# IvanBanny/para-ortho-pca-bo

Hardware: AMD Instinct MI355X
Metric: BO iterations/sec (incl. GP refit + EI opt), BBOB f15 d=40 (higher is better)
Workload: dtype f64; 1 GPU; configs[1]: PCA_BO on BBOB f15 d=40, budget=450, n_DoE=120, EI, var_threshold=0.95; one run per GPU (run list f15/d40/instances 0..N-1 partitioned by pcabo.sharding), timed steps spread evenly over the 330 BO iterations of the run; num_restarts=10, raw_samples=512, batch_limit=5, maxiter=200, parallelism=run-parallel x1

## Files before the change

### para-ortho-pca-bo_amd/csrc/kernels_acq.hip

```cpp
#include "pcabo_internal.h"
#include <algorithm>
#include <cstdlib>
#include <mutex>

#define PSTRIDE (2 + 2 * PCABO_MAXD)

#ifdef PCABO_ACQ_TIMING
__device__ unsigned long long g_acq_stamps[16];
#define STAMP(i) do { if (blockIdx.x == gridDim.x / 2 && blockIdx.y == 0 && threadIdx.x == 0) g_acq_stamps[i] = wall_clock64(); } while (0)
#define STAMP_FIN(i) do { if (blockIdx.y == 0 && threadIdx.x == 0) g_acq_stamps[i] = wall_clock64(); } while (0)
extern "C" int pcabo_debug_acq_stamps(unsigned long long* out16) {
  return hipMemcpyFromSymbol(out16, HIP_SYMBOL(g_acq_stamps), sizeof(g_acq_stamps)) == hipSuccess ? 0 : -3;
}
#else
#define STAMP(i)
#define STAMP_FIN(i)
#endif

__device__ inline void st_wt(double* p, double v) {
  __hip_atomic_store(p, v, __ATOMIC_RELAXED, __HIP_MEMORY_SCOPE_AGENT);
}

template <int SLAB>
__device__ inline int slab_row(int s, int m, int NP) {
// ... 23 lines not shown
    for (int t = 0; t < 8; ++t) {
      const int si = sl + 3 * t;
      const int sc = si < S ? si : 0;
      a[t] = base[(size_t)sc * PSTRIDE + 2 + c];
      b[t] = base[(size_t)sc * PSTRIDE + 2 + PCABO_MAXD + c];
    }
#pragma unroll
    for (int t = 0; t < 8; ++t) { if (sl + 3 * t < S) { gs += a[t]; gm += b[t]; } }
  }
  *gs_out = gs;
  *gm_out = gm;
}

__device__ void acq_finish_scalar(const double* base, int S, int q, const double* ystats, const AcqParams& p, double* val,
                                  double* host_val, double* coef, int lane);
__device__ void acq_scalar_core(double vv, double mus, int q, double ym, double ysd, const AcqParams& p, double* val,
                                double* host_val, double* coef, int l);
template <int SLAB>
__device__ inline void acq_tail(int combine, double* s_v, double* partial, unsigned int* counters, int q, int S, int k,
                                const double* bounds4, const double* ystats, const AcqParams& prm, double* val,
                                double* grad, double* host_val, double* host_grad, HostMirror* hm,
                                unsigned long long seq, int tid, int w, int l) {
  if (!combine) return;
  int* s_flag = reinterpret_cast<int*>(s_v + SLAB);
  STAMP(6);
  asm volatile("s_waitcnt vmcnt(0)" ::: "memory");
  __syncthreads();
  STAMP(7);
  if (tid == 0) {
    unsigned int t = __hip_atomic_fetch_add(&counters[q], 1u, __ATOMIC_RELAXED, __HIP_MEMORY_SCOPE_AGENT);
    int last = ((t % (unsigned int)S) == (unsigned int)(S - 1));
    if (last) {
// ... 56 lines not shown
    counters = zrun(counters, ab.zs, run_); val = zrun(val, ab.zs, run_); grad = zrun(grad, ab.zs, run_);        \
    Xq = zrun(Xq, ab.xq_host ? ab.hzs : ab.zs, run_);                                                            \
    host_val = zrun(host_val, ab.hzs, run_); host_grad = zrun(host_grad, ab.hzs, run_); hm = zrun(hm, ab.hzs, run_); \
    if (ab.k_dev) k = *zrun(ab.k_dev, ab.zs, run_);                                                              \
    if (ab.bestf) prm.best_f = *zrun(ab.bestf, ab.zs, run_);                                                     \
  }                                                                                                              \
  (void)qsel_;

template <int SLAB>
__global__ __launch_bounds__(256) void k_acq_fused(
    QueryArgs qa, const double* __restrict__ Xq, int q_total, int n, int k, int NP, int ld,
    const double* __restrict__ ZnT, const double* __restrict__ R, const double* __restrict__ alpha,
    const double* __restrict__ bounds4, const double* __restrict__ ystats, AcqParams prm, double* partial,
    unsigned int* counters, double* __restrict__ val, double* __restrict__ grad,
    double* host_val, double* host_grad, HostMirror* hm, unsigned long long seq, int combine, int ,
    MailPair* , MailPair* , AcqBatch ab) {
  ACQ_BATCH_PROLOGUE()
  const double inv_ls = prm.inv_ls;
  const int kernel = prm.kernel, want_grad = prm.want_grad;
  extern __shared__ __attribute__((aligned(16))) double s_dyn[];
  double* s_ks = s_dyn;
  double* s_cf = s_dyn + NP;
  double* s_tm = s_dyn + 2 * NP;
  double* s_xn = s_dyn + 3 * NP;
  double* s_v = s_xn + PCABO_MAXD;
  const int tid = threadIdx.x, w = tid >> 6, l = tid & 63;
  const int s = blockIdx.x, q = ab.table ? qsel_ : (int)blockIdx.y, S = gridDim.x;
  double* out = partial + ((size_t)q * S + s) * PSTRIDE;
  STAMP(0);

  if (tid < k) {
// ... 98 lines not shown
    if (l == 0) {
#pragma unroll
      for (int u = 0; u < 8; ++u) {
        const int c = c0 + w + 4 * u;
        if (c < k) { st_wt(out + 2 + c, gs[u]); st_wt(out + 2 + PCABO_MAXD + c, gm[u]); }
      }
    }
  }
  }

  acq_tail<SLAB>(combine, s_v, partial, counters, q, S, k, bounds4, ystats, prm, val, grad, host_val, host_grad, hm, seq, tid, w, l);
}

#define FIN_STAGE_PER_WAVE (11 * 2 * 40)
__device__ inline bool acq_server_finisher(const MailPair* rec, int S, int k, int q, unsigned long long seq,
                                           const double* ystats, const AcqParams& prm, double* val, double* grad,
                                           double* host_val, double* host_grad, HostMirror* hm, double rng_c,
                                           double* s_fin, double* s_coef, double* s_stage, int* s_srv,
                                           unsigned long long t0, int w, int l) {
  if (w == 0) {
    const double ym = ystats[0], ysd = ystats[1];
    const void* ptr[8];
    pcabo_u4 o[8];
    const MailPair* mine = rec + (size_t)(l < S ? l : 0) * PSTRIDE;
#pragma unroll
    for (int t = 0; t < 8; ++t) ptr[t] = mine + (t & 1);
    for (;;) {
      ld_pairs_sys8(ptr, o);
      const bool ok = pair_tag(o[0]) == seq && pair_tag(o[1]) == seq;
      if (__all(ok)) break;
      if (__any(wall_clock64() - t0 > PCABO_SERVER_TIMEOUT_TICKS)) { if (l == 0) *s_srv = 1; break; }
      __builtin_amdgcn_s_sleep(1);
    }
    double vm[2] = {l < S ? pair_value(o[0]) : 0.0, l < S ? pair_value(o[1]) : 0.0};
    wave_sum_multi<2>(vm, l);
    constexpr int lane_vv = wave_multi_lane(2, 0), lane_mus = wave_multi_lane(2, 1);
    const double vv = read_lane(vm[0], lane_vv), mus = read_lane(vm[0], lane_mus);
    acq_scalar_core(vv, mus, q, ym, ysd, prm, val, host_val, s_coef, l);
  } else if (prm.want_grad) {
    const int first = w - 1;
    const int ns = first < S ? (S - first + 2) / 3 : 0;
    const int total = ns * 2 * k;
    double* stage = s_stage + (size_t)(w - 1) * FIN_STAGE_PER_WAVE;
    for (int i0 = 0; i0 < total; i0 += 512) {
      const void* ptr[8];
      int item[8];
#pragma unroll
      for (int t = 0; t < 8; ++t) {
        const int i = i0 + l + 64 * t;
        item[t] = i < total ? i : -1;
        const int ii = i < total ? i : 0;
        const int st = ii / (2 * k), rem = ii - st * 2 * k, which = rem >= k, c = rem - which * k;
        ptr[t] = rec + (size_t)(first + 3 * st) * PSTRIDE + 2 + which * PCABO_MAXD + c;
      }
// ... 11 lines not shown
      for (int t = 0; t < 8; ++t) if (item[t] >= 0) stage[item[t]] = pair_value(o[t]);
    }
    __builtin_amdgcn_fence(__ATOMIC_RELEASE, "wavefront");
    __builtin_amdgcn_wave_barrier();
    __builtin_amdgcn_fence(__ATOMIC_ACQUIRE, "wavefront");
    if (l < k) {
      double gs = 0.0, gm = 0.0;
      for (int st = 0; st < ns; ++st) { gs += stage[st * 2 * k + l]; gm += stage[st * 2 * k + k + l]; }
      s_fin[(w - 1) * 2 * PCABO_MAXD + l] = gs;
      s_fin[(w - 1) * 2 * PCABO_MAXD + PCABO_MAXD + l] = gm;
    }
  }
  __syncthreads();
  if (*s_srv) return false;
  if (w == 0) {
    if (prm.want_grad && l < k) {
      const double c_mu = s_coef[0], c_sg = s_coef[1];
      const double gs = (s_fin[l] + s_fin[2 * PCABO_MAXD + l]) + s_fin[4 * PCABO_MAXD + l];
      const double gm = (s_fin[PCABO_MAXD + l] + s_fin[3 * PCABO_MAXD + l]) + s_fin[5 * PCABO_MAXD + l];
      const double g = __fma_rn(c_mu, gm, c_sg * gs) / rng_c;
      grad[(size_t)q * k + l] = g;
      if (host_grad) host_grad[(size_t)q * k + l] = g;
    }
    if (hm && l == 0)
      __hip_atomic_store(const_cast<unsigned long long*>(&hm->qflag[q]), seq, __ATOMIC_RELEASE, __HIP_MEMORY_SCOPE_SYSTEM);
  }
  return true;
}

#define FIN_LDS_DOUBLES (6 * PCABO_MAXD + 2 + 3 * FIN_STAGE_PER_WAVE + 2)
__device__ __noinline__ void acq_server_finish_main(double* s_mem, MailPair* dev_mail,
                                                    int ctrl_idx, const MailPair* part_pairs, int S, int k, int q,
                                                    const double* __restrict__ bounds4, const double* __restrict__ ystats,
                                                    const AcqParams& prm, double* val, double* grad, double* host_val,
                                                    double* host_grad, HostMirror* hm, unsigned long long seq) {
  double* s_fin = s_mem;
  int* s_srvp = reinterpret_cast<int*>(s_mem + FIN_LDS_DOUBLES - 1);
  const int tid = threadIdx.x, l = tid & 63;
  const int w = __builtin_amdgcn_readfirstlane(tid >> 6);
  double rng_c = 1.0;
  if (tid < k) rng_c = bounds4[PCABO_MAXD + tid] - bounds4[tid];
  for (unsigned long long cur_seq = seq;; ++cur_seq) {
    const unsigned long long t0 = wall_clock64();
    if (tid == 0) { s_srvp[0] = 0; s_srvp[1] = 0; }
    __syncthreads();
    if (w == 0) {
      for (;;) {
        const pcabo_u4 hd = ld_pair_sys(dev_mail + ctrl_idx);
        if (__all(mail_seq(hd) == cur_seq)) { if (pair_value(hd) == 0.0 && l == 0) *s_srvp = 1; break; }
        if (__any(wall_clock64() - t0 > PCABO_SERVER_TIMEOUT_TICKS)) { if (l == 0) *s_srvp = 1; break; }
        __builtin_amdgcn_s_sleep(1);
      }
    }
    __syncthreads();
    if (*s_srvp) return;
    if (!acq_server_finisher(part_pairs + (size_t)q * S * PSTRIDE, S, k, q, cur_seq, ystats, prm, val, grad, host_val,
                             host_grad, hm, rng_c, s_fin, s_fin + 6 * PCABO_MAXD, s_fin + 6 * PCABO_MAXD + 2, s_srvp, t0, w, l))
      return;
    __syncthreads();
  }
}

#define ACQ_SLAB32_NP 448
int acq_slabs(int NP) { return NP / (NP >= ACQ_SLAB32_NP ? 32 : 16); }

template <int NU, int CU>
__device__ inline void publish_grad(const double (&gs)[CU], const double (&gm)[CU], int w, int k, int l, MailPair* pout,
                                    double* out, unsigned long long seq) {
  static_assert(NU <= CU, "components per wave");
  double v[2 * NU];
#pragma unroll
  for (int u = 0; u < NU; ++u) { v[2 * u] = gs[u]; v[2 * u + 1] = gm[u]; }
// ... 2 lines not shown
  const int c = w + 4 * (i >> 1);
  if (i >= 0 && c < k) {
    const int off = 2 + (i & 1) * PCABO_MAXD + c;
    if (pout) st_pair_sys(pout + off, make_pair(v[0], seq));
    else st_wt(out + off, v[0]);
  }
}

template <int SLAB, int NB, bool SRV>
__global__ __launch_bounds__(256) void k_acq_fast(
    QueryArgs qa, const double* __restrict__ Xq, int q_total, int n, int k, int NP_rt, int ld,
    const double* __restrict__ ZnT, const double* __restrict__ R, const double* __restrict__ alpha,
    const double* __restrict__ bounds4, const double* __restrict__ ystats, AcqParams prm, double* partial,
    unsigned int* counters, double* __restrict__ val, double* __restrict__ grad,
    double* host_val, double* host_grad, HostMirror* hm, unsigned long long seq, int combine, int qb,
    MailPair* dev_mail, MailPair* part_pairs, AcqBatch ab) {
  if (!SRV) { ACQ_BATCH_PROLOGUE() }
  constexpr int NP = NB * 64;
  constexpr int CU = 10;
  constexpr int RW = SLAB / 4;
  constexpr int NM = (NB + 3) / 4;
  const double inv_ls = prm.inv_ls;
  const int kernel = prm.kernel, want_grad = prm.want_grad;
  extern __shared__ __attribute__((aligned(16))) double s_dyn[];
  double* s_ks = s_dyn;
  double* s_cf = s_dyn + NP;
  double* s_tm = s_dyn + 2 * NP;
  double* s_xn = s_dyn + 3 * NP;
  double* s_v = s_xn + PCABO_MAXD;
  double* s_p4 = s_v + SLAB + 2;
  const int tid = threadIdx.x, l = tid & 63;
  const int w = __builtin_amdgcn_readfirstlane(tid >> 6);
  constexpr bool server = SRV;
  const int s = blockIdx.x, S = server ? (int)gridDim.x - 1 : (int)gridDim.x;
  if (server && s == S) {
    acq_server_finish_main(s_dyn, dev_mail, 1 + q_total * k + (int)blockIdx.y, part_pairs, S, k,
                           blockIdx.y, bounds4, ystats, prm, val, grad, host_val, host_grad, hm, seq);
    return;
  }
  STAMP(0);

  double z[CU][NB], r[RW][NB], al[NM];
  const unsigned lane8 = (unsigned)l * 8u;
#pragma unroll
  for (int u = 0; u < CU; ++u) {
    const int c = w + 4 * u;
    const char* zr = reinterpret_cast<const char*>(ZnT + (size_t)c * ld);
#pragma unroll
    for (int b = 0; b < NB; ++b) {
      z[u][b] = 0.0;
      if (c < k) z[u][b] = *reinterpret_cast<const double*>(zr + lane8 + 512 * b);
    }
// ... 205 lines not shown
    return;
  }
  double log_phi = -0.5 * (u * u + log2pi);
  if (u > -1e6) {
    const double ex = erfcx(-inv_sqrt2 * u);
    const double E = (ex * fabs(u)) * 1.2533141373155003;
    *h = log_phi + log1p(-E);
    const double dw = (u + 0.7978845608028654 / ex) + 1.0 / u;
    *dh = -u - dw * E / (1.0 - E);
  } else {
    *h = log_phi - 2.0 * log(fabs(u));
    *dh = -u - 2.0 / u;
  }
}

__device__ void acq_scalar_core(double vv, double mus, int q, double ym, double ysd, const AcqParams& p, double* val,
                                double* host_val, double* coef, int l) {
  const double mu = ym + ysd * mus;
  double var = (1.0 - vv) * (ysd * ysd);
  bool clamped = false;
  if (!(var >= 1e-10)) { var = 1e-10; clamped = true; }
  if (var < 1e-12) { var = 1e-12; clamped = true; }
  const double sigma = sqrt(var);
  double u = (mu - p.best_f) / sigma;
  const double sgn = p.maximize ? 1.0 : -1.0;
  u *= sgn;
  double value, dv_du, dv_dsig;
  if (p.acq == 0) {
    double h, dh;
    log_ei_helper(u, &h, &dh);
    value = h + log(sigma);
    dv_du = dh;
    dv_dsig = 1.0 / sigma;
  } else {
    value = 0.5 * erfc(-0.7071067811865476 * u);
    dv_du = 0.3989422804014327 * exp(-0.5 * u * u);
    dv_dsig = 0.0;
  }
  if (l == 0) {
    val[q] = value;
    if (host_val) host_val[q] = value;
    coef[0] = dv_du * sgn * ysd / sigma;
    coef[1] = clamped ? 0.0 : (dv_dsig - dv_du * u / sigma) * (-(ysd * ysd) / sigma);
  }
  STAMP_FIN(12);
}

__device__ void acq_finish_scalar(const double* base, int S, int q, const double* ystats, const AcqParams& p, double* val,
                                  double* host_val, double* coef, int l) {
  const double ym = ystats[0], ysd = ystats[1];
  double vv = 0.0, mus = 0.0;
  for (int s = l; s < S; s += 64) { vv += base[(size_t)s * PSTRIDE]; mus += base[(size_t)s * PSTRIDE + 1]; }
  vv = wave_sum(vv);
  mus = wave_sum(mus);
  STAMP_FIN(11);
  acq_scalar_core(vv, mus, q, ym, ysd, p, val, host_val, coef, l);
}

__device__ void acq_finish_query(const double* base, int S, int k, int q, const double* bounds4, const double* ystats,
                                 const AcqParams& p, double* val, double* grad, double* host_val, double* host_grad,
// ... 572 lines not shown
bool acq_server_possible(int q, int n, int k, int NP) {
  static int cus = -1;
  if (cus < 0) {
    int dev = 0;
    if (hipGetDevice(&dev) != hipSuccess || hipDeviceGetAttribute(&cus, hipDeviceAttributeMultiprocessorCount, dev) != hipSuccess) cus = 0;
  }
  if (k > 40 || NP > 512 || q < 1 || q > PCABO_INLAUNCH_MAXQ || (size_t)q * k > PCABO_QA_MAX) return false;
  const int S = acq_slabs(NP);
  return (S + 1) * q <= cus && S <= 32;
}

void launch_acq(hipStream_t st, const QueryArgs* qa, const double* Xq, int q, int n, int k, int NP, int ld,
                const double* ZnT, const double* R, const double* alpha, const double* bounds4, const double* ystats,
                AcqParams p, double* partial, unsigned int* counters, double* val,
                double* grad, double* host_val, double* host_grad, HostMirror* hm, unsigned long long seq,
                MailPair* dev_mail, MailPair* part_pairs, AcqBatch ab, int B,
                int table_entries) {
  const int slab = NP >= ACQ_SLAB32_NP ? 32 : 16;
  const int S = NP / slab;
  static const QueryArgs empty = {};
  const int combine = hm != nullptr;
  const int nb = NP / 64;
  const bool fast = k <= 40 && nb <= 8;
  const int qb = (fast && !combine && q >= 64) ? 8 : 1;
  const int gy = ab.table ? table_entries : (q + qb - 1) / qb;
  const int gz = ab.table ? 1 : B;
#define ACQ_ARGS qa ? *qa : empty, Xq, q, n, k, NP, ld, ZnT, R, alpha, bounds4, ystats, p, partial, counters, val, grad, \
                 host_val, host_grad, hm, seq, combine, qb, dev_mail, part_pairs, ab
  const int FIN_LDS = 6 * PCABO_MAXD + 2;
#define ACQ_LDS(SL, NBV) (3 * NBV * 64 + PCABO_MAXD + SL + 2 + (4 * NBV * 64 > FIN_LDS ? 4 * NBV * 64 : FIN_LDS))
#define ACQ_FAST(SL, NBV)                                                                                      \
  case NBV:                                                                                                    \
    if (dev_mail)                                                                                              \
      hipLaunchKernelGGL((k_acq_fast<SL, NBV, true>), dim3(S + 1, gy), dim3(256),                              \
                         (size_t)std::max<int>(ACQ_LDS(SL, NBV), FIN_LDS_DOUBLES) * sizeof(double), st, ACQ_ARGS); \
    else                                                                                                       \
      hipLaunchKernelGGL((k_acq_fast<SL, NBV, false>), dim3(S, gy, gz), dim3(256),                             \
                         (size_t)ACQ_LDS(SL, NBV) * sizeof(double), st, ACQ_ARGS);                             \
    break;
  if (fast) {
    if (slab == 16) {
      switch (nb) { ACQ_FAST(16, 1) ACQ_FAST(16, 2) ACQ_FAST(16, 3) ACQ_FAST(16, 4) ACQ_FAST(16, 5) ACQ_FAST(16, 6)
                    ACQ_FAST(16, 7) ACQ_FAST(16, 8) }
// ... 59 lines not shown
```

### para-ortho-pca-bo_amd/csrc/pcabo_api.hip

```cpp
#include "../../include/pcabo.h"
#include "pcabo_internal.h"
#include "lbfgsb.h"
#include "host_side.h"

#include <algorithm>
#include <atomic>
#include <chrono>
#include <thread>
#include <condition_variable>
#include <functional>
#include <mutex>
#include <cstdlib>
#include <cmath>
#include <cstdio>
#include <cstring>
#include <new>
#include <vector>
#include <dirent.h>
#include <fcntl.h>
#include <signal.h>
#include <stdint.h>
#include <cerrno>
#include <unistd.h>
#include <emmintrin.h>
// ... 73 lines not shown
  unsigned int* dCounters = nullptr;
  int cnt_S = 0; bool cnt_dirty = true;
  double* dKS = nullptr;
  double* dBestF = nullptr;
  double* dMll = nullptr;
  char *dRegion = nullptr, *hRegion = nullptr;
  size_t region_bytes = 0, hregion_bytes = 0;
  bool in_batch = false; int batch_index = 0;
  bool rt_stale = false;
  HostMirror* hm = nullptr;
  double *hXq = nullptr, *hVal = nullptr, *hGrad = nullptr, *hSmall = nullptr, *hBestF = nullptr;
  double* hMll = nullptr;
  MailPair* dMail = nullptr;
  bool mail_bar = false;
  MailPair* dPairs = nullptr;
  bool opt_resident = true;
  bool opt_group_acq = false;
  bool bestf_f32 = true;
  int srv_penalty = 0;
  unsigned long long seq = 0;
  OptHelper helper;
  std::vector<std::unique_ptr<OptHelper>> more_helpers;
  bool registered = false;
  bool alone = true; int alone_age = 0;
  char err[512] = {0};
  bool prof = false;
  std::vector<ProfPair> pairs;
  size_t pairs_used = 0;
  double prof_ms[PROF_GROUPS] = {0};
  double prof_pair_ms = 0.0;
// ... 265 lines not shown
    HIPCHK(hipHostMalloc((void**)&ctx->hRegion, ctx->hregion_bytes, hipHostMallocDefault));
    memset(ctx->hRegion, 0, ctx->hregion_bytes);
  }
  carve_device(ctx, ctx->dRegion);
  carve_host(ctx, ctx->hRegion);
  if (!dreg) {
    HIPCHK(hipMemsetAsync(ctx->dRegion, 0, ctx->region_bytes, ctx->stream));
    if (hipExtMallocWithFlags((void**)&ctx->dMail, PCABO_MAIL_PAIRS * sizeof(MailPair), hipDeviceMallocFinegrained) != hipSuccess) {
      (void)hipGetLastError();
      HIPCHK(dalloc(&ctx->dMail, PCABO_MAIL_PAIRS));
    }
    HIPCHK(hipMemsetAsync(ctx->dMail, 0, PCABO_MAIL_PAIRS * sizeof(MailPair), ctx->stream));
    const size_t np = (size_t)PCABO_INLAUNCH_MAXQ * 32 * (2 + 2 * PCABO_MAXD);
    HIPCHK(dalloc(&ctx->dPairs, np));
    HIPCHK(hipMemsetAsync(ctx->dPairs, 0, np * sizeof(MailPair), ctx->stream));
    HIPCHK(hipStreamSynchronize(ctx->stream));
    ctx->mail_bar = mail_bar_usable(ctx);
  } else {
    ctx->opt_resident = false;
  }
  {
    static std::atomic<unsigned long long> ctx_counter{0};
    ctx->seq = ((unsigned long long)(getpid() & 0xffff) << 44) + ((ctx_counter.fetch_add(1) + 1) << 30);
  }
  return PCABO_OK;
}

static void ctx_teardown(pcabo_ctx* ctx) {
  (void)hipSetDevice(ctx->device);
  if (ctx->stream) (void)hipStreamSynchronize(ctx->stream);
  for (auto& p : ctx->pairs) { (void)hipEventDestroy(p.a); (void)hipEventDestroy(p.b); }
  if (!ctx->in_batch) {
    if (ctx->dRegion) (void)hipFree(ctx->dRegion);
    if (ctx->hRegion) (void)hipHostFree(ctx->hRegion);
    if (ctx->dMail) (void)hipFree(ctx->dMail);
    if (ctx->dPairs) (void)hipFree(ctx->dPairs);
  }
  if (ctx->evBounds) (void)hipEventDestroy(ctx->evBounds);
  if (ctx->evPca) (void)hipEventDestroy(ctx->evPca);
  if (ctx->stream && !ctx->in_batch) (void)hipStreamDestroy(ctx->stream);
  ctx->helper.shutdown();
  for (auto& h : ctx->more_helpers) h->shutdown();
  ctx->more_helpers.clear();
  if (ctx->registered) presence_unregister(ctx->device);
}

static bool ctx_sizes_ok(int max_n, int max_d, int max_q) {
  return max_n >= 2 && max_d >= 1 && max_d <= PCABO_MAXD && max_q >= 1 && max_q < PCABO_CNT_DONE;
}

extern "C" {
// ... 559 lines not shown
  memcpy(val, ctx->hVal, (size_t)q * sizeof(double));
  return PCABO_OK;
}

int pcabo_logei(pcabo_ctx* ctx, const double* Xq, int q, double best_f, int maximize, double* val, double* grad) {
  return pcabo_acq_eval(ctx, Xq, q, best_f, maximize, PCABO_ACQ_LOG_EI, val, grad);
}

static void server_post(pcabo_ctx* ctx, int cap, int nq, int k, unsigned long long tag) {
  MailPair* m = ctx->dMail;
  const int np = cap * k;
  for (int i = 0; i < np; ++i) put_mail_pair(m + 1 + i, ctx->hXq[i], tag);
  for (int q = 0; q < cap; ++q) put_mail_pair(m + 1 + np + q, q < nq ? 1.0 : 0.0, tag);
  _mm_sfence();
}
static int server_wait(pcabo_ctx* ctx, int nq, unsigned long long tag) {
  if (wait_flags(ctx->hm, 0, nq, tag, deadline_in(3)) != FLAGS_SET)
    return set_err(ctx, PCABO_ERR_TIMEOUT, "resident acquisition kernel did not answer%s", "");
  return PCABO_OK;
}

int pcabo_optimize_acqf(pcabo_ctx* ctx, const double* ics, int num_restarts, int batch_limit, const double* bounds,
                        int maxiter, double best_f, int maximize, int acq, double* cand, double* vals, int* info,
                        int* failed) {
  if (!ctx) return PCABO_ERR_ARG;
  if (!ics || !bounds || !cand || !vals || num_restarts < 1 || batch_limit < 1 || num_restarts > ctx->max_q ||
      (acq != PCABO_ACQ_LOG_EI && acq != PCABO_ACQ_PI))
    return set_err(ctx, PCABO_ERR_ARG, "pcabo_optimize_acqf: bad argument%s", "");
  if (!ctx->have_gp) return set_err(ctx, PCABO_ERR_ARG, "pcabo_optimize_acqf: call pcabo_gp_condition first%s", "");
  HIPCHK(hipSetDevice(ctx->device));
  const int k = ctx->k;
  RunRestarts run;
// ... 45 lines not shown
    for (int gi = 0; gi < ngroups; ++gi) {
      qoff[gi] = -1;
      if (!grp[gi].active) continue;
      qoff[gi] = nq;
      memcpy(ctx->hXq + (size_t)nq * k, grp[gi].x.data(), grp[gi].x.size() * sizeof(double));
      nq += grp[gi].nq;
    }
    if (nq == 0) break;
    int rc;
    if (round_no == 1 && (ctx->alone_age++ & 7) == 0) ctx->alone = presence_alone(ctx->device);
    const bool only_context_here = presence_local_contexts(ctx->device) == 1;
    if (round_no == 1 && ctx->srv_penalty > 0) --ctx->srv_penalty;
    else if (round_no == 1 && ctx->opt_resident && ctx->mail_bar && !ctx->opt_group_acq && ctx->alone && only_context_here && !ctx->prof && acq_server_possible(nq, ctx->n, k, ctx->NP)) {
      srv_cap = nq;
      launch_acq(ctx->stream, nullptr, nullptr, srv_cap, ctx->n, k, ctx->NP, ctx->ld, ctx->dZnT, ctx->dR, ctx->dAlpha,
                 ctx->dBounds4, ctx->dYstats, p, ctx->dPartial, ctx->dCounters, ctx->dVal, ctx->dGrad, ctx->hVal, ctx->hGrad,
                 ctx->hm, ctx->seq + 1, ctx->dMail, ctx->dPairs);
      HIPCHK(hipGetLastError());
      if (ngroups == 2 && grp[0].active && grp[1].active && nq == num_restarts) {
        const unsigned long long seq0 = ctx->seq;
        MailPair* m = ctx->dMail;
        const int cap = srv_cap;
        std::atomic<int> abort_flag{0};
        int timed_out[2] = {0, 0}, got_nan[2] = {0, 0}, left[2] = {0, 0}, slow_first[2] = {0, 0};
        unsigned long long used[2] = {0, 0};
        auto free_loop = [&](int gi) {
          RestartGroup& rg = grp[gi];
          const int q0 = rg.q0, nqg = rg.nq;
          unsigned long long r = 0;
          for (;;) {
            if (abort_flag.load(std::memory_order_relaxed)) { pending[gi] = 1; break; }
            const unsigned long long tag = seq0 + (++r);
            for (int t = 0; t < nqg * k; ++t) put_mail_pair(m + 1 + q0 * k + t, rg.x[t], tag);
            for (int j = 0; j < nqg; ++j) put_mail_pair(m + 1 + cap * k + q0 + j, 1.0, tag);
            _mm_sfence();
            const auto t0 = std::chrono::steady_clock::now();
            unsigned long spins = 0;
            bool ok = true;
            for (int j = 0; j < nqg && ok; ++j) {
              while (__atomic_load_n(&ctx->hm->qflag[q0 + j], __ATOMIC_ACQUIRE) != tag) {
                if ((++spins & 0xFFF) == 0) {
                  if (abort_flag.load(std::memory_order_relaxed)) { ok = false; break; }
                  if (std::chrono::steady_clock::now() - t0 > std::chrono::seconds(3)) {
                    timed_out[gi] = 1; abort_flag.store(1, std::memory_order_relaxed); ok = false; break;
                  }
                }
              }
            }
            if (!ok) { pending[gi] = 1; break; }
            if (r == 1 && std::chrono::steady_clock::now() - t0 > std::chrono::milliseconds(1)) slow_first[gi] = 1;
            if (!rg.absorb(ctx->hVal, ctx->hGrad, q0)) { got_nan[gi] = 1; abort_flag.store(1, std::memory_order_relaxed); break; }
            if (!rg.advance()) break;
          }
          const unsigned long long bye = seq0 + r + 1;
          for (int j = 0; j < nqg; ++j) put_mail_pair(m + 1 + cap * k + q0 + j, 0.0, bye);
          _mm_sfence();
          left[gi] = 1;
          used[gi] = r + 1;
        };
        hp.fn = [&] { free_loop(1); };
        const unsigned fticket = hp.go.load(std::memory_order_relaxed) + 1;
        hp.go.store(fticket, std::memory_order_release);
        free_loop(0);
        while (hp.done.load(std::memory_order_acquire) != fticket) __builtin_ia32_pause();
        hp.fn = [&] { for (int gi = 1; gi < ngroups; gi += T) advance(gi); };
        HIPCHK(hipStreamSynchronize(ctx->stream));
        ctx->seq = seq0 + std::max(used[0], used[1]) + 1;
        srv_cap = 0;
        if (got_nan[0] || got_nan[1]) return set_err(ctx, PCABO_ERR_NAN, "NaN in acquisition gradient%s", "");
        if (timed_out[0] || timed_out[1]) ctx->srv_penalty = 1000;
        else if (slow_first[0] || slow_first[1]) ctx->srv_penalty = 40;
        if (!grp[0].active && !grp[1].active) break;
        continue;
      }
    }
    if (srv_cap > 0) {
      const unsigned long long tag = ++ctx->seq;
      const double tp = now();
      server_post(ctx, srv_cap, nq, k, tag);
      rc = server_wait(ctx, nq, tag);
      if (rc == PCABO_ERR_TIMEOUT) {
        server_stop.stop();
        ctx->srv_penalty = 1000;
        rc = eval_staged(ctx, nq, p);
      } else if (round_no == 1 && now() - tp > 1e-3) {
        ctx->srv_penalty = 40;
      }
    } else if (group_mode(ctx, nq, 1) && batch_limit <= PCABO_GROUP_Q && ngroups <= 8) {
      int g0[8], gn[8], ng = 0;
      for (int gi = 0; gi < ngroups; ++gi) if (qoff[gi] >= 0) { g0[ng] = qoff[gi]; gn[ng] = grp[gi].nq; ++ng; }
      rc = eval_staged_groups(ctx, g0, gn, ng, p);
    } else {
      rc = eval_staged(ctx, nq, p);
    }
    if (rc != PCABO_OK) return rc;
// ... 548 lines not shown
  const int B = batch->B, kmax = batch_max_k(batch);
  pcabo_ctx* c0 = batch->ctx[0];
  if (phase != 2) {
  for (int b = 0; b < B; ++b)
    memcpy(batch->ctx[b]->hXq, Xq + (size_t)b * q * batch->max_d, (size_t)q * batch->ctx[b]->k * sizeof(double));
  BHIPCHK(hipMemcpy2DAsync(c0->dXq, batch->zs, c0->hXq, batch->hzs, (size_t)q * kmax * sizeof(double), B, hipMemcpyHostToDevice, s));
  int rc = batch_put_best_f(batch, best_f);
  if (rc != PCABO_OK) return rc;
  AcqParams p = make_params(c0, 0.0, maximize, acq, 0);
  p.inv_ls = 1.0 / batch->lengthscale; p.kernel = batch->kernel;
  if (score_gemm_possible(q))
    launch_score(s, c0->dXq, q, batch->n, kmax, batch->NP, c0->ld, c0->dZnT, c0->dR, c0->dAlpha, c0->dBounds4, c0->dYstats, p,
                 c0->dKS, c0->dPartial, c0->dVal, batch_ab(batch, 0, 0), B);
  else
    launch_acq(s, nullptr, c0->dXq, q, batch->n, kmax, batch->NP, c0->ld, c0->dZnT, c0->dR, c0->dAlpha, c0->dBounds4, c0->dYstats,
               p, c0->dPartial, c0->dCounters, c0->dVal, c0->dGrad, nullptr, nullptr, nullptr, 0, nullptr, nullptr,
               batch_ab(batch, 0, 0), B, 0);
  BHIPCHK(hipMemcpy2DAsync(c0->hVal, batch->hzs, c0->dVal, batch->zs, (size_t)q * sizeof(double), B, hipMemcpyDeviceToHost, s));
  BHIPCHK(hipGetLastError());
  batch->score_enqueued = true;
  }
  if (phase == 1) return PCABO_OK;
  BHIPCHK(wait_stream(s));
  BHIPCHK(hipGetLastError());
  batch->score_enqueued = false;
  batch->gp_pending = false; batch->have_gp = true;
  int worst = PCABO_OK;
  for (int b = 0; b < B; ++b) {
    pcabo_ctx* c = batch->ctx[b];
    int st = PCABO_OK;
    if (c->hm->chol_info != 0) {
// ... 243 lines not shown
    QueryArgs tab;
    unsigned* ent = reinterpret_cast<unsigned*>(tab.x);
    int nent = 0;
    auto launch = [&](const AcqParams& p, bool groups) -> bool {
      const unsigned long long seq = batch->seq.fetch_add(1) + 1;
      const int n = nent;
      nent = 0;
      if (groups) {
        if (launch_acq_group(st, &tab, n, c0->hXq, batch->n, kmax, batch->NP, c0->ld, c0->dZnT, c0->dR, c0->dAlpha,
                             c0->dBounds4, c0->dYstats, p, c0->dPartial, c0->dCounters + PCABO_GROUP_CNT_OFFSET, c0->dVal,
                             c0->dGrad, c0->hVal, c0->hGrad, c0->hm, seq, batch_ab(batch, 1, 1)) != 0)
          return false;
      } else {
        launch_acq(st, &tab, c0->hXq, PCABO_INLAUNCH_MAXQ, batch->n, kmax, batch->NP, c0->ld, c0->dZnT, c0->dR,
                   c0->dAlpha, c0->dBounds4, c0->dYstats, p, c0->dPartial, c0->dCounters, c0->dVal, c0->dGrad, c0->hVal,
                   c0->hGrad, c0->hm, seq, nullptr, nullptr, batch_ab(batch, 1, 1), B, n);
      }
      if (hipGetLastError() != hipSuccess) return false;
      const auto deadline = deadline_in(20);
      for (int e = 0; e < n; ++e) {
        const unsigned u = ent[e];
        const int q0 = groups ? (int)((u >> 8) & 0xffu) : (int)(u & 0xffffu), nq = groups ? (int)(u & 0xffu) : 1;
        if (wait_flags(batch->ctx[u >> 16]->hm, q0, nq, seq, deadline) != FLAGS_SET) return false;
      }
      return true;
    };
    auto stage = [&](int b, const RestartGroup& rg) {
      if (use_group) ent[nent++] = group_entry(b, rg.q0, rg.nq);
      else for (int j = 0; j < rg.nq; ++j) ent[nent++] = query_entry(b, rg.q0 + j);
    };
    const int rc = run_rounds(runs.data(), mine, stage, [&] { return launch(pg, use_group) ? PCABO_OK : PCABO_ERR_HIP; });
// ... 250 lines not shown
```

### para-ortho-pca-bo_amd/csrc/pcabo_internal.h

```cpp
#pragma once
#include <hip/hip_runtime.h>
#include <stdint.h>
#include <type_traits>

#define PCABO_BS 64
#define PCABO_SLAB 16
#define PCABO_MAXD 128
#define PCABO_TLD 66

#define PCABO_QA_MAX 416
#define PCABO_CNT_DONE 0x3fff
#define PCABO_INLAUNCH_MAXQ 32

typedef double double4_t __attribute__((ext_vector_type(4)));
struct QueryArgs { double x[PCABO_QA_MAX]; };
struct alignas(16) MailPair { double v; unsigned long long tag; };
static inline __host__ __device__ unsigned long long mail_mix(unsigned long long vbits) {
  const unsigned int lo = (unsigned int)vbits, hi = (unsigned int)(vbits >> 32);
  return (unsigned long long)((lo ^ hi ^ (hi >> 11)) & 0xFFFFFFu);
}
#define PCABO_MAIL_PAIRS (1 + PCABO_QA_MAX + PCABO_INLAUNCH_MAXQ + 1)
#define PCABO_SERVER_TIMEOUT_TICKS 200000000ull

#ifdef __HIPCC__
__device__ inline double fast_rcp(double x) {
  double r = __builtin_amdgcn_rcp(x);
  r = fma(fma(-x, r, 1.0), r, r);
  r = fma(fma(-x, r, 1.0), r, r);
  return r;
}
__device__ inline double fast_rsq(double x) {
  double y = __builtin_amdgcn_rsq(x);
  y = y * fma(-0.5 * x * y, y, 1.5);
  y = y * fma(-0.5 * x * y, y, 1.5);
  return y;
}
// ... 43 lines not shown
  asm volatile(
      "global_load_dwordx4 %0, %8, off sc0 sc1\n\tglobal_load_dwordx4 %1, %9, off sc0 sc1\n\t"
      "global_load_dwordx4 %2, %10, off sc0 sc1\n\tglobal_load_dwordx4 %3, %11, off sc0 sc1\n\t"
      "global_load_dwordx4 %4, %12, off sc0 sc1\n\tglobal_load_dwordx4 %5, %13, off sc0 sc1\n\t"
      "global_load_dwordx4 %6, %14, off sc0 sc1\n\tglobal_load_dwordx4 %7, %15, off sc0 sc1\n\t"
      "s_waitcnt vmcnt(0)"
      : "=&v"(o[0]), "=&v"(o[1]), "=&v"(o[2]), "=&v"(o[3]), "=&v"(o[4]), "=&v"(o[5]), "=&v"(o[6]), "=&v"(o[7])
      : "v"(p[0]), "v"(p[1]), "v"(p[2]), "v"(p[3]), "v"(p[4]), "v"(p[5]), "v"(p[6]), "v"(p[7])
      : "memory");
}
__device__ inline pcabo_u4 make_pair(double v, unsigned long long tag) {
  pcabo_u4 r;
  r.x = (unsigned int)__double2loint(v); r.y = (unsigned int)__double2hiint(v);
  r.z = (unsigned int)(tag & 0xffffffffull); r.w = (unsigned int)(tag >> 32);
  return r;
}
__device__ inline unsigned long long pair_tag(pcabo_u4 v) { return ((unsigned long long)v.w << 32) | v.z; }
__device__ inline double pair_value(pcabo_u4 v) { return __hiloint2double((int)v.y, (int)v.x); }
__device__ inline unsigned long long mail_seq(pcabo_u4 v) {
  return pair_tag(v) ^ mail_mix(((unsigned long long)v.y << 32) | v.x);
}

template <typename T>
__device__ inline T* zrun(T* p, size_t stride, unsigned run) {
  typedef typename std::remove_const<T>::type U;
  return p ? reinterpret_cast<T*>(reinterpret_cast<char*>(const_cast<U*>(p)) + (size_t)run * stride) : p;
}
#define ZRUN(p) p = zrun(p, zs, blockIdx.z)

struct XcdTile { unsigned run, x, y; };
// ... 134 lines not shown
                 ZB zb = ZB());
void launch_add_jitter(hipStream_t s, double* K, int n, int ld, double jitter);
int launch_cholesky(hipStream_t s, double* L, int NP, int ld, int* info, double* diag_scratch, ZB zb = ZB());
void launch_trinv(hipStream_t s, const double* L, int NP, int ld, double* R, ZB zb = ZB());
void launch_chol_panel(hipStream_t s, double* L, int p, int nblocks, int ld, int* info, double* diag_scratch, ZB zb = ZB());
int launch_chol_steps(hipStream_t s, double* L, int NP, int ld, int* info, double* diag_scratch , ZB zb = ZB());
void launch_trinv_diag_w(hipStream_t s, const double* L, int nblk, int ld, double* R, ZB zb = ZB());
void launch_alpha(hipStream_t s, const double* R, const double* ys, int n, int NP, int ld, double* tmp, double* alpha,
                  ZB zb = ZB());
void launch_mll_grad(hipStream_t s, const double* R, const double* AT, const double* nrm, const double* alpha, const double* L,
                     const double* ys, int n, int NP, int KP, int ld, double* partial, double* out);
void launch_acq(hipStream_t s, const QueryArgs* qa, const double* Xq, int q, int n, int k, int NP, int ld,
                const double* ZnT, const double* R, const double* alpha, const double* bounds4, const double* ystats,
                AcqParams p, double* partial, unsigned int* counters, double* val,
                double* grad, double* host_val, double* host_grad, HostMirror* hm, unsigned long long seq,
                MailPair* dev_mail = nullptr, MailPair* part_pairs = nullptr,
                AcqBatch ab = AcqBatch(), int B = 1, int table_entries = 0);
#define PCABO_GROUP_Q 5
#define PCABO_GROUP_CNT_OFFSET 8192
bool acq_group_possible(int NP, int k);
int launch_acq_group(hipStream_t st, const QueryArgs* tab, int entries, const double* Xq, int n, int k, int NP, int ld,
                     const double* ZnT, const double* R, const double* alpha, const double* bounds4, const double* ystats,
                     AcqParams p, double* partial, unsigned int* counters, double* val, double* grad, double* host_val,
                     double* host_grad, HostMirror* hm, unsigned long long seq, AcqBatch ab);
bool score_gemm_possible(int q);
void launch_score(hipStream_t st, const double* Xq, int q, int n, int k, int NP, int ld, const double* ZnT, const double* R,
                  const double* alpha, const double* bounds4, const double* ystats, AcqParams p, double* KS, double* partial,
                  double* val, AcqBatch ab = AcqBatch(), int B = 1);
bool acq_server_possible(int q, int n, int k, int NP);
int acq_slabs(int NP);
void launch_inverse_map(hipStream_t s, const double* z, const double* comps, const double* data_mean,
// ... 9 lines not shown
```

Before: 383.2 BO iterations/s.

## Return resident acquisition results as tagged pairs in host memory

The resident server finisher now writes each acquisition value and gradient element to a pinned host buffer as a self-validating (value, seq-mixed tag) pair. It no longer writes device val/grad plus host mirrors and then publishes a release-ordered qflag. The host polls these tagged pairs directly, removing the separate flag store and its fence ordering from the per-query response path. In exchange the host must spin on one pair per gradient element rather than a single flag, and it relies on 16-byte stores arriving atomically over the system bus.

```diff
diff --git a/para-ortho-pca-bo_amd/csrc/kernels_acq.hip b/para-ortho-pca-bo_amd/csrc/kernels_acq.hip
--- a/para-ortho-pca-bo_amd/csrc/kernels_acq.hip
+++ b/para-ortho-pca-bo_amd/csrc/kernels_acq.hip
@@ -61,8 +61,8 @@
 
 __device__ void acq_finish_scalar(const double* base, int S, int q, const double* ystats, const AcqParams& p, double* val,
                                   double* host_val, double* coef, int lane);
-__device__ void acq_scalar_core(double vv, double mus, int q, double ym, double ysd, const AcqParams& p, double* val,
-                                double* host_val, double* coef, int l);
+__device__ double acq_scalar_core(double vv, double mus, int q, double ym, double ysd, const AcqParams& p, double* val,
+                                  double* host_val, double* coef, int l);
 template <int SLAB>
 __device__ inline void acq_tail(int combine, double* s_v, double* partial, unsigned int* counters, int q, int S, int k,
                                 const double* bounds4, const double* ystats, const AcqParams& prm, double* val,
@@ -149,7 +149,7 @@
     const double* __restrict__ bounds4, const double* __restrict__ ystats, AcqParams prm, double* partial,
     unsigned int* counters, double* __restrict__ val, double* __restrict__ grad,
     double* host_val, double* host_grad, HostMirror* hm, unsigned long long seq, int combine, int ,
-    MailPair* , MailPair* , AcqBatch ab) {
+    MailPair* , MailPair* , MailPair* , AcqBatch ab) {
   ACQ_BATCH_PROLOGUE()
   const double inv_ls = prm.inv_ls;
   const int kernel = prm.kernel, want_grad = prm.want_grad;
@@ -278,8 +278,8 @@
 
 #define FIN_STAGE_PER_WAVE (11 * 2 * 40)
 __device__ inline bool acq_server_finisher(const MailPair* rec, int S, int k, int q, unsigned long long seq,
-                                           const double* ystats, const AcqParams& prm, double* val, double* grad,
-                                           double* host_val, double* host_grad, HostMirror* hm, double rng_c,
+                                           const double* ystats, const AcqParams& prm, int want_grad, MailPair* res,
+                                           double rng_c,
                                            double* s_fin, double* s_coef, double* s_stage, int* s_srv,
                                            unsigned long long t0, int w, int l) {
   if (w == 0) {
@@ -300,8 +300,9 @@
     wave_sum_multi<2>(vm, l);
     constexpr int lane_vv = wave_multi_lane(2, 0), lane_mus = wave_multi_lane(2, 1);
     const double vv = read_lane(vm[0], lane_vv), mus = read_lane(vm[0], lane_mus);
-    acq_scalar_core(vv, mus, q, ym, ysd, prm, val, host_val, s_coef, l);
-  } else if (prm.want_grad) {
+    const double value = acq_scalar_core(vv, mus, q, ym, ysd, prm, nullptr, nullptr, s_coef, l);
+    if (l == 0) st_pair_sys(res, make_mail_pair(value, seq));
+  } else if (want_grad) {
     const int first = w - 1;
     const int ns = first < S ? (S - first + 2) / 3 : 0;
     const int total = ns * 2 * k;
@@ -343,16 +344,13 @@
   __syncthreads();
   if (*s_srv) return false;
   if (w == 0) {
-    if (prm.want_grad && l < k) {
+    if (want_grad && l < k) {
       const double c_mu = s_coef[0], c_sg = s_coef[1];
       const double gs = (s_fin[l] + s_fin[2 * PCABO_MAXD + l]) + s_fin[4 * PCABO_MAXD + l];
       const double gm = (s_fin[PCABO_MAXD + l] + s_fin[3 * PCABO_MAXD + l]) + s_fin[5 * PCABO_MAXD + l];
       const double g = __fma_rn(c_mu, gm, c_sg * gs) / rng_c;
-      grad[(size_t)q * k + l] = g;
-      if (host_grad) host_grad[(size_t)q * k + l] = g;
-    }
-    if (hm && l == 0)
-      __hip_atomic_store(const_cast<unsigned long long*>(&hm->qflag[q]), seq, __ATOMIC_RELEASE, __HIP_MEMORY_SCOPE_SYSTEM);
+      st_pair_sys(res + 1 + l, make_mail_pair(g, seq));
+    }
   }
   return true;
 }
@@ -361,14 +359,14 @@
 __device__ __noinline__ void acq_server_finish_main(double* s_mem, MailPair* dev_mail,
                                                     int ctrl_idx, const MailPair* part_pairs, int S, int k, int q,
                                                     const double* __restrict__ bounds4, const double* __restrict__ ystats,
-                                                    const AcqParams& prm, double* val, double* grad, double* host_val,
-                                                    double* host_grad, HostMirror* hm, unsigned long long seq) {
+                                                    const AcqParams& prm, MailPair* res, unsigned long long seq) {
   double* s_fin = s_mem;
   int* s_srvp = reinterpret_cast<int*>(s_mem + FIN_LDS_DOUBLES - 1);
   const int tid = threadIdx.x, l = tid & 63;
   const int w = __builtin_amdgcn_readfirstlane(tid >> 6);
   double rng_c = 1.0;
   if (tid < k) rng_c = bounds4[PCABO_MAXD + tid] - bounds4[tid];
+  const int want_grad = __builtin_amdgcn_readfirstlane(prm.want_grad);
   for (unsigned long long cur_seq = seq;; ++cur_seq) {
     const unsigned long long t0 = wall_clock64();
     if (tid == 0) { s_srvp[0] = 0; s_srvp[1] = 0; }
@@ -383,8 +381,8 @@
     }
     __syncthreads();
     if (*s_srvp) return;
-    if (!acq_server_finisher(part_pairs + (size_t)q * S * PSTRIDE, S, k, q, cur_seq, ystats, prm, val, grad, host_val,
-                             host_grad, hm, rng_c, s_fin, s_fin + 6 * PCABO_MAXD, s_fin + 6 * PCABO_MAXD + 2, s_srvp, t0, w, l))
+    if (!acq_server_finisher(part_pairs + (size_t)q * S * PSTRIDE, S, k, q, cur_seq, ystats, prm, want_grad, res, rng_c, s_fin,
+                             s_fin + 6 * PCABO_MAXD, s_fin + 6 * PCABO_MAXD + 2, s_srvp, t0, w, l))
       return;
     __syncthreads();
   }
@@ -417,7 +415,7 @@
     const double* __restrict__ bounds4, const double* __restrict__ ystats, AcqParams prm, double* partial,
     unsigned int* counters, double* __restrict__ val, double* __restrict__ grad,
     double* host_val, double* host_grad, HostMirror* hm, unsigned long long seq, int combine, int qb,
-    MailPair* dev_mail, MailPair* part_pairs, AcqBatch ab) {
+    MailPair* dev_mail, MailPair* part_pairs, MailPair* res_pairs, AcqBatch ab) {
   if (!SRV) { ACQ_BATCH_PROLOGUE() }
   constexpr int NP = NB * 64;
   constexpr int CU = 10;
@@ -438,7 +436,7 @@
   const int s = blockIdx.x, S = server ? (int)gridDim.x - 1 : (int)gridDim.x;
   if (server && s == S) {
     acq_server_finish_main(s_dyn, dev_mail, 1 + q_total * k + (int)blockIdx.y, part_pairs, S, k,
-                           blockIdx.y, bounds4, ystats, prm, val, grad, host_val, host_grad, hm, seq);
+                           blockIdx.y, bounds4, ystats, prm, res_pairs + (size_t)blockIdx.y * PCABO_RES_STRIDE, seq);
     return;
   }
   STAMP(0);
@@ -674,8 +672,8 @@
   }
 }
 
-__device__ void acq_scalar_core(double vv, double mus, int q, double ym, double ysd, const AcqParams& p, double* val,
-                                double* host_val, double* coef, int l) {
+__device__ double acq_scalar_core(double vv, double mus, int q, double ym, double ysd, const AcqParams& p, double* val,
+                                  double* host_val, double* coef, int l) {
   const double mu = ym + ysd * mus;
   double var = (1.0 - vv) * (ysd * ysd);
   bool clamped = false;
@@ -698,12 +696,13 @@
     dv_dsig = 0.0;
   }
   if (l == 0) {
-    val[q] = value;
+    if (val) val[q] = value;
     if (host_val) host_val[q] = value;
     coef[0] = dv_du * sgn * ysd / sigma;
     coef[1] = clamped ? 0.0 : (dv_dsig - dv_du * u / sigma) * (-(ysd * ysd) / sigma);
   }
   STAMP_FIN(12);
+  return value;
 }
 
 __device__ void acq_finish_scalar(const double* base, int S, int q, const double* ystats, const AcqParams& p, double* val,
@@ -1306,19 +1305,19 @@
                 const double* ZnT, const double* R, const double* alpha, const double* bounds4, const double* ystats,
                 AcqParams p, double* partial, unsigned int* counters, double* val,
                 double* grad, double* host_val, double* host_grad, HostMirror* hm, unsigned long long seq,
-                MailPair* dev_mail, MailPair* part_pairs, AcqBatch ab, int B,
+                MailPair* dev_mail, MailPair* part_pairs, MailPair* res_pairs, AcqBatch ab, int B,
                 int table_entries) {
   const int slab = NP >= ACQ_SLAB32_NP ? 32 : 16;
   const int S = NP / slab;
   static const QueryArgs empty = {};
-  const int combine = hm != nullptr;
+  const int combine = hm != nullptr || dev_mail != nullptr;
   const int nb = NP / 64;
   const bool fast = k <= 40 && nb <= 8;
   const int qb = (fast && !combine && q >= 64) ? 8 : 1;
   const int gy = ab.table ? table_entries : (q + qb - 1) / qb;
   const int gz = ab.table ? 1 : B;
 #define ACQ_ARGS qa ? *qa : empty, Xq, q, n, k, NP, ld, ZnT, R, alpha, bounds4, ystats, p, partial, counters, val, grad, \
-                 host_val, host_grad, hm, seq, combine, qb, dev_mail, part_pairs, ab
+                 host_val, host_grad, hm, seq, combine, qb, dev_mail, part_pairs, res_pairs, ab
   const int FIN_LDS = 6 * PCABO_MAXD + 2;
 #define ACQ_LDS(SL, NBV) (3 * NBV * 64 + PCABO_MAXD + SL + 2 + (4 * NBV * 64 > FIN_LDS ? 4 * NBV * 64 : FIN_LDS))
 #define ACQ_FAST(SL, NBV)                                                                                      \
diff --git a/para-ortho-pca-bo_amd/csrc/pcabo_api.hip b/para-ortho-pca-bo_amd/csrc/pcabo_api.hip
--- a/para-ortho-pca-bo_amd/csrc/pcabo_api.hip
+++ b/para-ortho-pca-bo_amd/csrc/pcabo_api.hip
@@ -111,6 +111,7 @@
   MailPair* dMail = nullptr;
   bool mail_bar = false;
   MailPair* dPairs = nullptr;
+  MailPair* hRes = nullptr;
   bool opt_resident = true;
   bool opt_group_acq = false;
   bool bestf_f32 = true;
@@ -406,6 +407,8 @@
     const size_t np = (size_t)PCABO_INLAUNCH_MAXQ * 32 * (2 + 2 * PCABO_MAXD);
     HIPCHK(dalloc(&ctx->dPairs, np));
     HIPCHK(hipMemsetAsync(ctx->dPairs, 0, np * sizeof(MailPair), ctx->stream));
+    HIPCHK(hipHostMalloc((void**)&ctx->hRes, PCABO_RES_PAIRS * sizeof(MailPair), hipHostMallocDefault));
+    memset(ctx->hRes, 0, PCABO_RES_PAIRS * sizeof(MailPair));
     HIPCHK(hipStreamSynchronize(ctx->stream));
     ctx->mail_bar = mail_bar_usable(ctx);
   } else {
@@ -427,6 +430,7 @@
     if (ctx->hRegion) (void)hipHostFree(ctx->hRegion);
     if (ctx->dMail) (void)hipFree(ctx->dMail);
     if (ctx->dPairs) (void)hipFree(ctx->dPairs);
+    if (ctx->hRes) (void)hipHostFree(ctx->hRes);
   }
   if (ctx->evBounds) (void)hipEventDestroy(ctx->evBounds);
   if (ctx->evPca) (void)hipEventDestroy(ctx->evPca);
@@ -1016,8 +1020,36 @@
   for (int q = 0; q < cap; ++q) put_mail_pair(m + 1 + np + q, q < nq ? 1.0 : 0.0, tag);
   _mm_sfence();
 }
-static int server_wait(pcabo_ctx* ctx, int nq, unsigned long long tag) {
-  if (wait_flags(ctx->hm, 0, nq, tag, deadline_in(3)) != FLAGS_SET)
+static inline bool take_result_pair(const MailPair* p, unsigned long long seq, double* v) {
+  __asm__ __volatile__("" ::: "memory");
+  const __m128i x = _mm_load_si128(reinterpret_cast<const __m128i*>(p));
+  const unsigned long long vb = (unsigned long long)_mm_cvtsi128_si64(x);
+  const unsigned long long tag = (unsigned long long)_mm_cvtsi128_si64(_mm_unpackhi_epi64(x, x));
+  if ((tag ^ mail_mix(vb)) != seq) return false;
+  memcpy(v, &vb, 8);
+  return true;
+}
+extern "C" int pcabo_debug_take_result_pair(const void* pair, unsigned long long seq, double* v) {
+  return take_result_pair(static_cast<const MailPair*>(pair), seq, v) ? 1 : 0;
+}
+enum { RES_TIMEOUT = -1, RES_STOPPED = 0, RES_OK = 1 };
+static int wait_result_pairs(pcabo_ctx* ctx, int q0, int nq, int k, bool want_grad, unsigned long long seq,
+                             std::chrono::steady_clock::time_point deadline, const std::atomic<int>* stop = nullptr) {
+  unsigned long spins = 0;
+  const int per_q = want_grad ? 1 + k : 1;
+  for (int q = q0; q < q0 + nq; ++q)
+    for (int i = 0; i < per_q; ++i) {
+      double* dst = i == 0 ? ctx->hVal + q : ctx->hGrad + (size_t)q * k + (i - 1);
+      while (!take_result_pair(ctx->hRes + (size_t)q * PCABO_RES_STRIDE + i, seq, dst)) {
+        if ((++spins & 0xFFF) != 0) continue;
+        if (stop && stop->load(std::memory_order_relaxed)) return RES_STOPPED;
+        if (std::chrono::steady_clock::now() > deadline) return RES_TIMEOUT;
+      }
+    }
+  return RES_OK;
+}
+static int server_wait(pcabo_ctx* ctx, int nq, int k, bool want_grad, unsigned long long tag) {
+  if (wait_result_pairs(ctx, 0, nq, k, want_grad, tag, deadline_in(3)) != RES_OK)
     return set_err(ctx, PCABO_ERR_TIMEOUT, "resident acquisition kernel did not answer%s", "");
   return PCABO_OK;
 }
@@ -1093,8 +1125,8 @@
     else if (round_no == 1 && ctx->opt_resident && ctx->mail_bar && !ctx->opt_group_acq && ctx->alone && only_context_here && !ctx->prof && acq_server_possible(nq, ctx->n, k, ctx->NP)) {
       srv_cap = nq;
       launch_acq(ctx->stream, nullptr, nullptr, srv_cap, ctx->n, k, ctx->NP, ctx->ld, ctx->dZnT, ctx->dR, ctx->dAlpha,
-                 ctx->dBounds4, ctx->dYstats, p, ctx->dPartial, ctx->dCounters, ctx->dVal, ctx->dGrad, ctx->hVal, ctx->hGrad,
-                 ctx->hm, ctx->seq + 1, ctx->dMail, ctx->dPairs);
+                 ctx->dBounds4, ctx->dYstats, p, ctx->dPartial, ctx->dCounters, nullptr, nullptr, nullptr, nullptr,
+                 nullptr, ctx->seq + 1, ctx->dMail, ctx->dPairs, ctx->hRes);
       HIPCHK(hipGetLastError());
       if (ngroups == 2 && grp[0].active && grp[1].active && nq == num_restarts) {
         const unsigned long long seq0 = ctx->seq;
@@ -1114,19 +1146,9 @@
             for (int j = 0; j < nqg; ++j) put_mail_pair(m + 1 + cap * k + q0 + j, 1.0, tag);
             _mm_sfence();
             const auto t0 = std::chrono::steady_clock::now();
-            unsigned long spins = 0;
-            bool ok = true;
-            for (int j = 0; j < nqg && ok; ++j) {
-              while (__atomic_load_n(&ctx->hm->qflag[q0 + j], __ATOMIC_ACQUIRE) != tag) {
-                if ((++spins & 0xFFF) == 0) {
-                  if (abort_flag.load(std::memory_order_relaxed)) { ok = false; break; }
-                  if (std::chrono::steady_clock::now() - t0 > std::chrono::seconds(3)) {
-                    timed_out[gi] = 1; abort_flag.store(1, std::memory_order_relaxed); ok = false; break;
-                  }
-                }
-              }
-            }
-            if (!ok) { pending[gi] = 1; break; }
+            const int got = wait_result_pairs(ctx, q0, nqg, k, p.want_grad != 0, tag, t0 + std::chrono::seconds(3), &abort_flag);
+            if (got == RES_TIMEOUT) { timed_out[gi] = 1; abort_flag.store(1, std::memory_order_relaxed); }
+            if (got != RES_OK) { pending[gi] = 1; break; }
             if (r == 1 && std::chrono::steady_clock::now() - t0 > std::chrono::milliseconds(1)) slow_first[gi] = 1;
             if (!rg.absorb(ctx->hVal, ctx->hGrad, q0)) { got_nan[gi] = 1; abort_flag.store(1, std::memory_order_relaxed); break; }
             if (!rg.advance()) break;
@@ -1157,7 +1179,7 @@
       const unsigned long long tag = ++ctx->seq;
       const double tp = now();
       server_post(ctx, srv_cap, nq, k, tag);
-      rc = server_wait(ctx, nq, tag);
+      rc = server_wait(ctx, nq, k, p.want_grad != 0, tag);
       if (rc == PCABO_ERR_TIMEOUT) {
         server_stop.stop();
         ctx->srv_penalty = 1000;
@@ -1736,7 +1758,7 @@
                  c0->dKS, c0->dPartial, c0->dVal, batch_ab(batch, 0, 0), B);
   else
     launch_acq(s, nullptr, c0->dXq, q, batch->n, kmax, batch->NP, c0->ld, c0->dZnT, c0->dR, c0->dAlpha, c0->dBounds4, c0->dYstats,
-               p, c0->dPartial, c0->dCounters, c0->dVal, c0->dGrad, nullptr, nullptr, nullptr, 0, nullptr, nullptr,
+               p, c0->dPartial, c0->dCounters, c0->dVal, c0->dGrad, nullptr, nullptr, nullptr, 0, nullptr, nullptr, nullptr,
                batch_ab(batch, 0, 0), B, 0);
   BHIPCHK(hipMemcpy2DAsync(c0->hVal, batch->hzs, c0->dVal, batch->zs, (size_t)q * sizeof(double), B, hipMemcpyDeviceToHost, s));
   BHIPCHK(hipGetLastError());
@@ -2010,7 +2032,7 @@
       } else {
         launch_acq(st, &tab, c0->hXq, PCABO_INLAUNCH_MAXQ, batch->n, kmax, batch->NP, c0->ld, c0->dZnT, c0->dR,
                    c0->dAlpha, c0->dBounds4, c0->dYstats, p, c0->dPartial, c0->dCounters, c0->dVal, c0->dGrad, c0->hVal,
-                   c0->hGrad, c0->hm, seq, nullptr, nullptr, batch_ab(batch, 1, 1), B, n);
+                   c0->hGrad, c0->hm, seq, nullptr, nullptr, nullptr, batch_ab(batch, 1, 1), B, n);
       }
       if (hipGetLastError() != hipSuccess) return false;
       const auto deadline = deadline_in(20);
diff --git a/para-ortho-pca-bo_amd/csrc/pcabo_internal.h b/para-ortho-pca-bo_amd/csrc/pcabo_internal.h
--- a/para-ortho-pca-bo_amd/csrc/pcabo_internal.h
+++ b/para-ortho-pca-bo_amd/csrc/pcabo_internal.h
@@ -20,6 +20,8 @@
   return (unsigned long long)((lo ^ hi ^ (hi >> 11)) & 0xFFFFFFu);
 }
 #define PCABO_MAIL_PAIRS (1 + PCABO_QA_MAX + PCABO_INLAUNCH_MAXQ + 1)
+#define PCABO_RES_STRIDE (1 + PCABO_MAXD)
+#define PCABO_RES_PAIRS (PCABO_INLAUNCH_MAXQ * PCABO_RES_STRIDE)
 #define PCABO_SERVER_TIMEOUT_TICKS 200000000ull
 
 #ifdef __HIPCC__
@@ -93,6 +95,10 @@
   r.x = (unsigned int)__double2loint(v); r.y = (unsigned int)__double2hiint(v);
   r.z = (unsigned int)(tag & 0xffffffffull); r.w = (unsigned int)(tag >> 32);
   return r;
+}
+__device__ inline pcabo_u4 make_mail_pair(double v, unsigned long long seq) {
+  const unsigned long long vb = ((unsigned long long)(unsigned int)__double2hiint(v) << 32) | (unsigned int)__double2loint(v);
+  return make_pair(v, seq ^ mail_mix(vb));
 }
 __device__ inline unsigned long long pair_tag(pcabo_u4 v) { return ((unsigned long long)v.w << 32) | v.z; }
 __device__ inline double pair_value(pcabo_u4 v) { return __hiloint2double((int)v.y, (int)v.x); }
@@ -257,7 +263,7 @@
                 const double* ZnT, const double* R, const double* alpha, const double* bounds4, const double* ystats,
                 AcqParams p, double* partial, unsigned int* counters, double* val,
                 double* grad, double* host_val, double* host_grad, HostMirror* hm, unsigned long long seq,
-                MailPair* dev_mail = nullptr, MailPair* part_pairs = nullptr,
+                MailPair* dev_mail = nullptr, MailPair* part_pairs = nullptr, MailPair* res_pairs = nullptr,
                 AcqBatch ab = AcqBatch(), int B = 1, int table_entries = 0);
 #define PCABO_GROUP_Q 5
 #define PCABO_GROUP_CNT_OFFSET 8192
```

After: 388.1 BO iterations/s (median of 6 runs). No clear change (+1.3%).
